# mratsim/constantine

Measured on NVIDIA H100. Metric: bls12_381_g1_msm_throughput, higher is better.
Workload: dtype u32

## Files before the change

### constantine_b200/csrc/msm_affine.cuh

```cuda
#pragma once
#include "ec.cuh"
#include "field_inv.cuh"

namespace b200 {

constexpr int AFF_MAX_LEVELS = 8;
constexpr uint32_t AFF_NONE = 0xFFFFFFFFu;

static __global__ void k_bucket_bounds(const uint32_t* __restrict__ keys, size_t n, uint32_t no_key, uint32_t* head, uint32_t* tail) {
  size_t q = (size_t)blockIdx.x * blockDim.x + threadIdx.x;
  if (q >= n) return;
  const uint32_t key = keys[q];
  if (key >= no_key) return;
  if (q == 0 || keys[q - 1] != key) head[key] = (uint32_t)q;
  if (q + 1 == n || keys[q + 1] != key) tail[key] = (uint32_t)(q + 1);
}

constexpr int SCAN_THREADS = 256, SCAN_PER_THREAD = 4, SCAN_ITEMS = SCAN_THREADS * SCAN_PER_THREAD;

B200_DEV uint32_t block_exclusive_scan(uint32_t v, uint32_t& total, uint32_t* smem ) {
  const unsigned lane = threadIdx.x & 31u, warp = threadIdx.x >> 5;
  uint32_t inc = v;
#pragma unroll
  for (int d = 1; d < 32; d <<= 1) {
// ... 3 lines not shown
  __syncthreads();
  if (lane == 31u) smem[warp] = inc;
  __syncthreads();
  uint32_t base = 0, tot = 0;
#pragma unroll
  for (int w = 0; w < SCAN_THREADS / 32; w++) {
    const uint32_t s = smem[w];
    if ((unsigned)w < warp) base += s;
    tot += s;
  }
  total = tot;
  return base + inc - v;
}

B200_DEV uint32_t level_count(uint32_t n, int r) { return (n + (1u << r) - 1u) >> r; }

static __global__ void __launch_bounds__(SCAN_THREADS) k_level_blocksums(const uint32_t* __restrict__ head, const uint32_t* __restrict__ tail,
                                                                          uint32_t nb, int L, uint32_t nblk, uint32_t* blocksum ) {
  __shared__ uint32_t sm[SCAN_THREADS / 32 + 1];
  const uint32_t b0 = blockIdx.x * SCAN_ITEMS + threadIdx.x * SCAN_PER_THREAD;
  uint32_t cnt[SCAN_PER_THREAD];
#pragma unroll
  for (int k = 0; k < SCAN_PER_THREAD; k++) cnt[k] = (b0 + k < nb) ? tail[b0 + k] - head[b0 + k] : 0u;
  for (int r = 0; r <= L; r++) {
    uint32_t s = 0;
#pragma unroll
    for (int k = 0; k < SCAN_PER_THREAD; k++) s += level_count(cnt[k], r);
    uint32_t tot;
    block_exclusive_scan(s, tot, sm);
    if (threadIdx.x == 0) blocksum[(size_t)r * nblk + blockIdx.x] = tot;
  }
}

static __global__ void __launch_bounds__(SCAN_THREADS) k_level_scan(uint32_t* blocksum, uint32_t nblk, int L, uint32_t nb, uint32_t* off) {
  __shared__ uint32_t sm[SCAN_THREADS / 32 + 1];
  for (int r = 0; r <= L; r++) {
    uint32_t carry = 0;
    for (uint32_t base = 0; base < nblk; base += SCAN_THREADS) {
      const uint32_t i = base + threadIdx.x;
      const uint32_t v = (i < nblk) ? blocksum[(size_t)r * nblk + i] : 0u;
      uint32_t tot;
      const uint32_t ex = block_exclusive_scan(v, tot, sm);
      if (i < nblk) blocksum[(size_t)r * nblk + i] = carry + ex;
      carry += tot;
    }
    if (threadIdx.x == 0) off[(size_t)r * (nb + 1) + nb] = carry;
  }
}

static __global__ void __launch_bounds__(SCAN_THREADS) k_level_offsets(const uint32_t* __restrict__ head, const uint32_t* __restrict__ tail,
                                                                        uint32_t nb, int L, uint32_t nblk, const uint32_t* __restrict__ blocksum,
                                                                        uint32_t* off) {
  __shared__ uint32_t sm[SCAN_THREADS / 32 + 1];
  const uint32_t b0 = blockIdx.x * SCAN_ITEMS + threadIdx.x * SCAN_PER_THREAD;
  uint32_t cnt[SCAN_PER_THREAD];
#pragma unroll
  for (int k = 0; k < SCAN_PER_THREAD; k++) cnt[k] = (b0 + k < nb) ? tail[b0 + k] - head[b0 + k] : 0u;
  for (int r = 0; r <= L; r++) {
    uint32_t c[SCAN_PER_THREAD], s = 0;
#pragma unroll
    for (int k = 0; k < SCAN_PER_THREAD; k++) { c[k] = level_count(cnt[k], r); s += c[k]; }
    uint32_t tot;
    uint32_t ex = block_exclusive_scan(s, tot, sm) + blocksum[(size_t)r * nblk + blockIdx.x];
#pragma unroll
    for (int k = 0; k < SCAN_PER_THREAD; k++) {
      if (b0 + k < nb) off[(size_t)r * (nb + 1) + b0 + k] = ex;
      ex += c[k];
    }
  }
}

struct AffinePlan {
  uint2* plan0;
  uint32_t* plan[AFF_MAX_LEVELS];
  uint32_t* surv_keys;
  uint32_t* surv_vals;
};

static __global__ void k_affine_plan(const uint32_t* __restrict__ keys, const uint32_t* __restrict__ vals, size_t n, uint32_t no_key,
                                     const uint32_t* __restrict__ head, const uint32_t* __restrict__ tail,
                                     const uint32_t* __restrict__ off, uint32_t nb, int L, AffinePlan P) {
  size_t q = (size_t)blockIdx.x * blockDim.x + threadIdx.x;
  if (q >= n) return;
  const uint32_t b = keys[q];
  if (b >= no_key) return;
  const uint32_t h = head[b], i = (uint32_t)q - h, cnt = tail[b] - h;
  const size_t stride = (size_t)nb + 1;
  for (int r = 0; r < L; r++) {
    if (i & ((2u << r) - 1u)) break;
    const uint32_t p = off[(size_t)(r + 1) * stride + b] + (i >> (r + 1));
    const uint32_t s = i >> r;
    const bool has2 = s + 1u < level_count(cnt, r);
    if (r == 0) P.plan0[p] = make_uint2(vals[q], has2 ? vals[q + 1] : AFF_NONE);
    else P.plan[r][p] = (off[(size_t)r * stride + b] + s) | (has2 ? 0x80000000u : 0u);
  }
  if ((i & ((1u << L) - 1u)) == 0u) {
    const uint32_t ps = off[(size_t)L * stride + b] + (i >> L);
    P.surv_keys[ps] = b;
    P.surv_vals[ps] = ps;
  }
}

template <class T>
B200_DEV Aff<T> load_affine_rw(const uint32_t* base, size_t idx) {
  const uint32_t* p = base + idx * (2 * T::WORDS);
  Aff<T> a;
  load_words_rw(a.x, p);
  load_words_rw(a.y, p + T::WORDS);
  return a;
// ... 18 lines not shown
template <class T>
B200_DEV T scratch_load(const uint4* scratch, size_t threads, size_t tid, uint32_t j) {
  constexpr int V = T::WORDS / 4;
  T v;
#pragma unroll
  for (int k = 0; k < V; k++) {
    const uint4 w = scratch[((size_t)j * V + k) * threads + tid];
    v.set_word(4 * k + 0, w.x); v.set_word(4 * k + 1, w.y); v.set_word(4 * k + 2, w.z); v.set_word(4 * k + 3, w.w);
  }
  return v;
}

constexpr int PART_TILE = 1024, PART_THREADS = 256, PART_MAX = 8;

B200_DEV uint32_t pair_chunk(const uint2 task, uint32_t n_points, uint32_t P) {
  uint32_t idx = task.x & 0x7FFFFFFFu;
  if (task.y != AFF_NONE) { const uint32_t j = task.y & 0x7FFFFFFFu; if (j > idx) idx = j; }
  uint32_t q = (uint32_t)(((unsigned long long)idx * P) / n_points);
  return q < P ? q : P - 1u;
}

static __global__ void __launch_bounds__(PART_THREADS) k_part_count(const uint2* __restrict__ plan0, const uint32_t* __restrict__ total_ptr,
                                                                    uint32_t n_points, uint32_t P, uint32_t nblk, uint32_t* counts) {
  __shared__ uint32_t sm[PART_MAX];
  if (threadIdx.x < PART_MAX) sm[threadIdx.x] = 0;
  __syncthreads();
  const uint32_t total = *total_ptr;
  const uint32_t base = blockIdx.x * PART_TILE;
  uint32_t local[PART_MAX];
#pragma unroll
  for (int q = 0; q < PART_MAX; q++) local[q] = 0;
  for (uint32_t i = threadIdx.x; i < PART_TILE; i += PART_THREADS) {
// ... 57 lines not shown
      for (unsigned w = 0; w < warp; w++) before += warp_cnt[w][q];
      perm[run_base[q] + before + my_rank] = p;
    }
    __syncthreads();
    if (threadIdx.x < P) {
      uint32_t tot = 0;
      for (unsigned w = 0; w < PART_THREADS / 32; w++) tot += warp_cnt[w][threadIdx.x];
      run_base[threadIdx.x] += tot;
    }
    __syncthreads();
  }
}

enum PairKind { PAIR_COPY1 = 0, PAIR_COPY2 = 1, PAIR_INF = 2, PAIR_ADD = 3, PAIR_DBL = 4 };

struct PairTask {
  uint32_t a, b;
};
template <bool FIRST>
B200_DEV PairTask load_task(const void* plan, size_t p) {
  PairTask t;
  if constexpr (FIRST) {
    const uint2 v = reinterpret_cast<const uint2*>(plan)[p];
    t.a = v.x; t.b = v.y;
  } else {
    const uint32_t v = reinterpret_cast<const uint32_t*>(plan)[p];
    t.a = v & 0x7FFFFFFFu;
    t.b = (v >> 31) ? t.a + 1u : AFF_NONE;
  }
  return t;
}
template <class T, bool FIRST>
B200_DEV T load_x(const uint32_t* src, uint32_t ref) {
  T x;
  if constexpr (FIRST) load_words(x, src + (size_t)(ref & 0x7FFFFFFFu) * (2 * T::WORDS));
  else load_words_rw(x, src + (size_t)ref * (2 * T::WORDS));
  return x;
}
template <class T, bool FIRST>
B200_DEV void decode_y(T& y, uint32_t ref, bool& zero) {
  zero = y.is_zero();
  if constexpr (FIRST) y.cneg((ref >> 31) != 0);
}
template <class T, bool FIRST>
B200_DEV T load_y(const uint32_t* src, uint32_t ref, bool& zero) {
  T y;
  if constexpr (FIRST) load_words(y, src + (size_t)(ref & 0x7FFFFFFFu) * (2 * T::WORDS) + T::WORDS);
  else load_words_rw(y, src + (size_t)ref * (2 * T::WORDS) + T::WORDS);
  decode_y<T, FIRST>(y, ref, zero);
  return y;
}

template <class T>
B200_DEV int classify_pair(bool single, const T& x1, const T& y1, bool inf1, const T& x2, const T& y2, bool inf2, T& den) {
  if (single) return PAIR_COPY1;
  if (inf1) return PAIR_COPY2;
  if (inf2) return PAIR_COPY1;
  den = x2 - x1;
  if (!den.is_zero()) return PAIR_ADD;
  if (!(y1 == y2) || y1.is_zero()) return PAIR_INF;
  den = y1.dbl();
  return PAIR_DBL;
}

template <class T, bool FIRST>
B200_DEV void pair_factor(const uint32_t* src, uint32_t a, uint32_t b, const T& x1, const T& x2, T& run) {
  const bool single = b == AFF_NONE;
  T den = x2 - x1;
  bool contributes = !single;
  if (!single && (den.is_zero() || x1.is_zero() || x2.is_zero())) {
    bool z1, z2;
    const T y1 = load_y<T, FIRST>(src, a, z1), y2 = load_y<T, FIRST>(src, b, z2);
    const int kind = classify_pair(false, x1, y1, z1 && x1.is_zero(), x2, y2, z2 && x2.is_zero(), den);
    contributes = kind >= PAIR_ADD;
  }
  if (contributes) run = run.mul_u(den);
}

template <class T, class Prefix>
B200_DEV Aff<T> pair_result(const Aff<T>& P1, bool z1, const Aff<T>& P2, bool z2, bool single, uint32_t j, T& inv, Prefix prefix) {
  T den;
  const int kind = classify_pair(single, P1.x, P1.y, z1 && P1.x.is_zero(), P2.x, P2.y, z2 && P2.x.is_zero(), den);
  Aff<T> R;
  if (kind < PAIR_ADD) {
    if (kind == PAIR_COPY1) R = P1;
    else if (kind == PAIR_COPY2) R = P2;
    else { R.x = T::zero(); R.y = T::zero(); }
  } else {
    T inv_den = inv;
    if (j > 0) inv_den = inv.mul_u(prefix());
    inv = inv.mul_u(den);
    T num;
    if (kind == PAIR_ADD) num = P2.y - P1.y;
    else { const T xx = P1.x.sqr(); num = xx.dbl() + xx; }
    const T lam = num.mul_u(inv_den);
    R.x = lam.sqr_u() - P1.x - P2.x;
    R.y = lam.mul_u(P1.x - R.x) - P1.y;
// ... 7 lines not shown
#ifndef B200_AFF_MIN_BLOCKS
#define B200_AFF_MIN_BLOCKS 4
#endif

B200_DEV void prefetch_l2(const void* p) { asm volatile("prefetch.global.L2 [%0];" ::"l"(p)); }
B200_DEV void prefetch_span(const void* p, int bytes) {
  prefetch_l2(p);
  prefetch_l2((const char*)p + bytes - 1);
}
template <class T, bool FIRST>
B200_DEV void prefetch_point(const uint32_t* src, uint32_t ref) {
  const uint32_t idx = FIRST ? (ref & 0x7FFFFFFFu) : ref;
  prefetch_span(src + (size_t)idx * (2 * T::WORDS), 2 * T::WORDS * 4);
}

__host__ __device__ __forceinline__ size_t pair_rows(size_t slots, size_t threads) { return (slots + threads - 1) / threads; }

struct PairSlots {
  const uint32_t* perm;
  uint32_t total, M;
  B200_DEV PairSlots(const uint32_t* total_ptr, const uint32_t* perm_, const uint32_t* range, size_t threads) {
    const uint32_t range_begin = range ? range[0] : 0u;
    total = range ? range[1] - range[0] : *total_ptr;
    perm = perm_;
    if (perm) perm += range_begin;
    M = (uint32_t)pair_rows(total, threads);
  }
  B200_DEV size_t first(size_t tid) const { return (tid & ~(size_t)31) * M + (tid & 31u); }
  B200_DEV uint32_t count(size_t tid) const {
    const size_t f = first(tid);
    if (f >= total) return 0u;
    const uint32_t c = (uint32_t)(((size_t)total - f + 31) / 32);
    return c < M ? c : M;
  }
  B200_DEV size_t slot(size_t tid, uint32_t j) const {
    const size_t t = first(tid) + 32u * (size_t)j;
    return perm ? (size_t)perm[t] : t;
  }
};

template <class T, bool FIRST>
__global__ void __launch_bounds__(B200_AFF_THREADS, (T::WORDS <= 12) ? B200_AFF_MIN_BLOCKS : 1)
k_affine_pairs(const void* __restrict__ plan, const uint32_t* __restrict__ total_ptr, const uint32_t* src, uint32_t* dst, uint4* scratch,
               const uint32_t* __restrict__ perm = nullptr, const uint32_t* __restrict__ range = nullptr) {
  const size_t threads = (size_t)gridDim.x * blockDim.x;
  const size_t tid = (size_t)blockIdx.x * blockDim.x + threadIdx.x;
  const PairSlots S(total_ptr, perm, range, threads);
  const unsigned lane = threadIdx.x & 31u;
  if (S.count(tid - lane) == 0) return;
  const uint32_t cnt = S.count(tid);
  T run = T::one();
  {
    PairTask t_next = cnt ? load_task<FIRST>(plan, S.slot(tid, 0)) : PairTask{0u, AFF_NONE};
    T x1n = T::zero(), x2n = T::zero();
    if (cnt) {
      x1n = load_x<T, FIRST>(src, t_next.a);
      if (t_next.b != AFF_NONE) x2n = load_x<T, FIRST>(src, t_next.b);
    }
#pragma unroll 1
    for (uint32_t j = 0; j < cnt; j++) {
      const PairTask t = t_next;
      const T x1 = x1n, x2 = x2n;
      if (j + 1 < cnt) {
        t_next = load_task<FIRST>(plan, S.slot(tid, j + 1));
        x1n = load_x<T, FIRST>(src, t_next.a);
        if (t_next.b != AFF_NONE) x2n = load_x<T, FIRST>(src, t_next.b);
      }
      pair_factor<T, FIRST>(src, t.a, t.b, x1, x2, run);
      scratch_store(scratch, threads, tid, j, run);
    }
  }
  T inv = fe_inverse(run);
  size_t p_prev = cnt ? S.slot(tid, cnt - 1) : 0;
  PairTask t_prev = cnt ? load_task<FIRST>(plan, p_prev) : PairTask{0u, AFF_NONE};
#pragma unroll 1
  for (uint32_t jj = cnt; jj > 0; jj--) {
    const uint32_t j = jj - 1;
    const size_t p = p_prev;
    const PairTask t = t_prev;
    if (j > 0) {
      p_prev = S.slot(tid, j - 1);
      t_prev = load_task<FIRST>(plan, p_prev);
      prefetch_point<T, FIRST>(src, t_prev.a);
      if (t_prev.b != AFF_NONE) prefetch_point<T, FIRST>(src, t_prev.b);
      if (j > 1) {
        constexpr int V = T::WORDS / 4;
#pragma unroll
        for (int k = 0; k < V; k++) prefetch_l2(scratch + ((size_t)(j - 2) * V + k) * threads + tid);
      }
    }
    const bool single = t.b == AFF_NONE;
    Aff<T> P1, P2;
    bool z1 = false, z2 = false;
    P1.x = load_x<T, FIRST>(src, t.a);
    P1.y = load_y<T, FIRST>(src, t.a, z1);
    if (!single) {
      P2.x = load_x<T, FIRST>(src, t.b);
      P2.y = load_y<T, FIRST>(src, t.b, z2);
    } else {
      P2.x = T::zero(); P2.y = T::zero();
    }
    store_affine(dst, p, pair_result(P1, z1, P2, z2, single, j, inv, [&] { return scratch_load<T>(scratch, threads, tid, j - 1); }));
  }
}

#ifndef B200_AFF_WS_CONSUMERS
#define B200_AFF_WS_CONSUMERS 8
#endif
#ifndef B200_AFF_WS_STAGES
#define B200_AFF_WS_STAGES 2
#endif
constexpr int AFF_WS_CONSUMERS = B200_AFF_WS_CONSUMERS;
constexpr int AFF_WS_THREADS = 32 * (AFF_WS_CONSUMERS + 1);

template <class T>
struct AffRing {
  static constexpr bool USED = T::WORDS <= 12;
  static constexpr int V = T::WORDS / 4;
// ... 24 lines not shown
  for (int k = 0; k < T::WORDS / 4; k++) cp_async16(ring + (row + k) * 32 + lane, g + 4 * k);
}
template <class T>
B200_DEV T ring_load(const uint4* ring, int row, unsigned lane) {
  T v;
#pragma unroll
  for (int k = 0; k < T::WORDS / 4; k++) {
    const uint4 w = ring[(row + k) * 32 + lane];
    v.set_word(4 * k + 0, w.x); v.set_word(4 * k + 1, w.y); v.set_word(4 * k + 2, w.z); v.set_word(4 * k + 3, w.w);
  }
  return v;
}

template <class T, bool FIRST>
__global__ void __launch_bounds__(AFF_WS_THREADS, 1)
k_affine_pairs_ws(const void* __restrict__ plan, const uint32_t* __restrict__ total_ptr, const uint32_t* src, uint32_t* dst, uint4* scratch,
                  const uint32_t* __restrict__ perm = nullptr, const uint32_t* __restrict__ range = nullptr) {
  using RG = AffRing<T>;
  constexpr int V = RG::V, NC = AFF_WS_CONSUMERS, S1 = RG::S1, S2 = RG::S2;
  extern __shared__ __align__(16) unsigned char aff_ring_raw[];
  __shared__ uint64_t full1[NC][S1], empty1[NC][S1], full2[NC][S2], empty2[NC][S2], drained[NC];
  __shared__ uint32_t s_task[NC][S1][3][32];
  const unsigned lane = threadIdx.x & 31u, warp = threadIdx.x >> 5;
  if (threadIdx.x == 0) {
    for (int w = 0; w < NC; w++) {
      for (int s = 0; s < S1; s++) { mbar_init(&full1[w][s], 64); mbar_init(&empty1[w][s], 32); }
      for (int s = 0; s < S2; s++) { mbar_init(&full2[w][s], 64); mbar_init(&empty2[w][s], 32); }
      mbar_init(&drained[w], 32);
    }
  }
  __syncthreads();
  const size_t threads = (size_t)gridDim.x * NC * 32;
  const PairSlots S(total_ptr, perm, range, threads);
  uint4* const ring_base = reinterpret_cast<uint4*>(aff_ring_raw);

  if (warp == NC) {
    uint32_t n[NC], cnt[NC];
#pragma unroll
    for (int w = 0; w < NC; w++) {
      const size_t tid = ((size_t)blockIdx.x * NC + w) * 32 + lane;
      n[w] = S.count(tid - lane);
      cnt[w] = S.count(tid);
    }
    auto tid_of = [&](int w) { return ((size_t)blockIdx.x * NC + w) * 32 + lane; };
    auto src_of = [&](uint32_t ref) { return src + (size_t)(FIRST ? (ref & 0x7FFFFFFFu) : ref) * (2 * T::WORDS); };
    uint32_t ta[NC], tb[NC], tp[NC];
    auto fetch_task = [&](int w, uint32_t j) {
      const size_t p = S.slot(tid_of(w), j);
      const PairTask t = load_task<FIRST>(plan, p);
      ta[w] = t.a; tb[w] = t.b; tp[w] = (uint32_t)p;
    };
#pragma unroll
    for (int w = 0; w < NC; w++) if (cnt[w]) fetch_task(w, 0);
#pragma unroll 1
    for (uint32_t j = 0; j < n[0]; j++) {
      uint32_t ca[NC], cb[NC];
#pragma unroll
      for (int w = 0; w < NC; w++) { ca[w] = ta[w]; cb[w] = tb[w]; }
#pragma unroll
      for (int w = 0; w < NC; w++) if (j + 1 < cnt[w]) fetch_task(w, j + 1);
#pragma unroll
      for (int w = 0; w < NC; w++) {
        if (j >= n[w]) continue;
        const int s = (int)(j % S1);
        mbar_wait(&empty1[w][s], ((j / S1) & 1u) ^ 1u);
        uint4* ring = ring_base + (size_t)w * RG::ROWS * 32;
        if (j < cnt[w]) {
          s_task[w][s][0][lane] = ca[w];
          s_task[w][s][1][lane] = cb[w];
          ring_fetch<T>(ring, s * 2 * V, lane, src_of(ca[w]));
          if (cb[w] != AFF_NONE) ring_fetch<T>(ring, s * 2 * V + V, lane, src_of(cb[w]));
        }
        cp_async_arrive(&full1[w][s]);
        mbar_arrive(&full1[w][s]);
      }
    }
#pragma unroll
    for (int w = 0; w < NC; w++) if (n[w] && n[w] - 1 < cnt[w]) fetch_task(w, n[w] - 1);
#pragma unroll 1
    for (uint32_t jj = 0; jj < n[0]; jj++) {
      uint32_t ca[NC], cb[NC], cp[NC];
#pragma unroll
      for (int w = 0; w < NC; w++) { ca[w] = ta[w]; cb[w] = tb[w]; cp[w] = tp[w]; }
#pragma unroll
      for (int w = 0; w < NC; w++) if (jj + 1 < n[w] && n[w] - 2 - jj < cnt[w]) fetch_task(w, n[w] - 2 - jj);
#pragma unroll
      for (int w = 0; w < NC; w++) {
        if (jj >= n[w]) continue;
        if (jj == 0) mbar_wait(&drained[w], 0);
        const uint32_t j = n[w] - 1 - jj;
        const int s = (int)(jj % S2);
        mbar_wait(&empty2[w][s], ((jj / S2) & 1u) ^ 1u);
        uint4* ring = ring_base + (size_t)w * RG::ROWS * 32;
        if (j < cnt[w]) {
          s_task[w][s][0][lane] = ca[w];
          s_task[w][s][1][lane] = cb[w];
          s_task[w][s][2][lane] = cp[w];
          const int row = s * 5 * V;
          ring_fetch<T>(ring, row, lane, src_of(ca[w]));
          ring_fetch<T>(ring, row + V, lane, src_of(ca[w]) + T::WORDS);
          if (cb[w] != AFF_NONE) {
            ring_fetch<T>(ring, row + 2 * V, lane, src_of(cb[w]));
            ring_fetch<T>(ring, row + 3 * V, lane, src_of(cb[w]) + T::WORDS);
          }
          if (j > 0) {
#pragma unroll
            for (int k = 0; k < V; k++)
              cp_async16(ring + (row + 4 * V + k) * 32 + lane, scratch + ((size_t)(j - 1) * V + k) * threads + tid_of(w));
          }
        }
        cp_async_arrive(&full2[w][s]);
        mbar_arrive(&full2[w][s]);
      }
    }
    asm volatile("cp.async.wait_all;" ::: "memory");
    return;
  }

  const size_t tid = ((size_t)blockIdx.x * NC + warp) * 32 + lane;
  const uint32_t n = S.count(tid - lane), cnt = S.count(tid);
  if (n == 0) return;
  const uint4* ring = ring_base + (size_t)warp * RG::ROWS * 32;
  T run = T::one();
#pragma unroll 1
  for (uint32_t j = 0; j < n; j++) {
    const int s = (int)(j % S1);
    mbar_wait(&full1[warp][s], (j / S1) & 1u);
    const uint32_t a = s_task[warp][s][0][lane], b = s_task[warp][s][1][lane];
    const T x1 = ring_load<T>(ring, s * 2 * V, lane), x2 = ring_load<T>(ring, s * 2 * V + V, lane);
    mbar_arrive(&empty1[warp][s]);
    if (j >= cnt) continue;
    pair_factor<T, FIRST>(src, a, b, x1, x2, run);
    scratch_store(scratch, threads, tid, j, run);
  }
  mbar_arrive(&drained[warp]);
  T inv = fe_inverse(run);
#pragma unroll 1
  for (uint32_t jj = 0; jj < n; jj++) {
    const uint32_t j = n - 1 - jj;
    const int s = (int)(jj % S2);
    mbar_wait(&full2[warp][s], (jj / S2) & 1u);
    const int row = s * 5 * V;
    const uint32_t a = s_task[warp][s][0][lane], b = s_task[warp][s][1][lane], p = s_task[warp][s][2][lane];
    const bool single = b == AFF_NONE;
    Aff<T> P1, P2;
    P1.x = ring_load<T>(ring, row, lane);
    P1.y = ring_load<T>(ring, row + V, lane);
    P2.x = single ? T::zero() : ring_load<T>(ring, row + 2 * V, lane);
    P2.y = single ? T::zero() : ring_load<T>(ring, row + 3 * V, lane);
    const T pre = ring_load<T>(ring, row + 4 * V, lane);
    mbar_arrive(&empty2[warp][s]);
    if (j >= cnt) continue;
    bool z1, z2 = false;
    decode_y<T, FIRST>(P1.y, a, z1);
    if (!single) decode_y<T, FIRST>(P2.y, b, z2);
    store_affine(dst, p, pair_result(P1, z1, P2, z2, single, j, inv, [&] { return pre; }));
  }
}

template <class T>
struct PairKernel {
  static constexpr bool WS = AffRing<T>::USED;
  static constexpr int THREADS = WS ? AFF_WS_THREADS : B200_AFF_THREADS;
  static constexpr int SLOT_THREADS = WS ? 32 * AFF_WS_CONSUMERS : B200_AFF_THREADS;
  static constexpr int SMEM = WS ? (int)AffRing<T>::BYTES : 0;
  template <bool FIRST>
  static auto entry() {
    if constexpr (WS) return k_affine_pairs_ws<T, FIRST>;
    else return k_affine_pairs<T, FIRST>;
  }
};

template <class T>
cudaError_t affine_pairs_blocks_per_sm(int* bps) {
  using K = PairKernel<T>;
  int b[2] = {0, 0};
  cudaError_t e;
  for (int f = 0; f < 2; f++) {
    const auto k = f == 0 ? K::template entry<true>() : K::template entry<false>();
    if (K::SMEM && (e = cudaFuncSetAttribute(k, cudaFuncAttributeMaxDynamicSharedMemorySize, K::SMEM)) != cudaSuccess) return e;
    if ((e = cudaOccupancyMaxActiveBlocksPerMultiprocessor(&b[f], k, K::THREADS, K::SMEM)) != cudaSuccess) return e;
  }
  *bps = b[1] < b[0] ? b[1] : b[0];
  return cudaSuccess;
}

template <class T, bool FIRST>
void launch_affine_pairs(unsigned grid, cudaStream_t s, const void* plan, const uint32_t* total_ptr, const uint32_t* src, uint32_t* dst, uint4* scratch,
                         const uint32_t* perm = nullptr, const uint32_t* range = nullptr) {
  using K = PairKernel<T>;
  K::template entry<FIRST>()<<<grid, K::THREADS, K::SMEM, s>>>(plan, total_ptr, src, dst, scratch, perm, range);
}

}
```

### constantine_b200/csrc/msm_engine.cuh

```cuda
#pragma once
#include <cstdio>
#include <cstdlib>
#include <cstring>
#include <atomic>
#include <condition_variable>
#include <functional>
#include <memory>
#include <mutex>
#include <thread>
#include <vector>
#include <cuda_runtime.h>
#include <cub/device/device_radix_sort.cuh>
#include <cub/device/device_scan.cuh>
#include "msm_kernels.cuh"
#include "msm_affine.cuh"
#include "host_field.hpp"

namespace b200 {

#define B200_CUDA_CHECK(expr)                                                                              \
  do {                                                                                                     \
    cudaError_t e__ = (expr);                                                                              \
    if (e__ != cudaSuccess) {                                                                              \
      fprintf(stderr, "[ctt_b200_msm] FATAL CUDA error %s (%s) at %s:%d -- no CPU fallback exists\n",      \
// ... 120 lines not shown
  int sm_count = 0;
  cudaStream_t stream = nullptr, copy_stream = nullptr;
  cudaStream_t user_stream = nullptr;
  cudaStream_t order_after = nullptr;
  cudaEvent_t ev_order = nullptr;
  cudaEvent_t ev_done = nullptr;
  bool unsynced = false, pending = false;
  cudaStream_t compute() const { return user_stream ? user_stream : stream; }
  cudaEvent_t msm_ev[MSM_MARKS];
  static constexpr int CALLER_MARKS = 6;
  cudaEvent_t caller_ev[CALLER_MARKS];
  cudaEvent_t ev_points_ready;
  static constexpr int MAX_INPUT_CHUNKS = 8;
  cudaEvent_t ev_chunk[MAX_INPUT_CHUNKS];
  DeviceBuffer d_scalars, d_points, keys_a, keys_b, vals_a, vals_b, cub_tmp, buckets, part_pts[2], part_keys[2], red_a, red_b, red_planes, bounds;
  DeviceBuffer aff_head, aff_tail, aff_off, aff_blocksum, aff_plan[AFF_MAX_LEVELS], aff_work[2], aff_scratch, keys_s, vals_s, part_counts, part_starts, part_perm;
  DeviceBuffer kzg_poly, kzg_args;
  DeviceBuffer das_coefs, das_cells, das_u, das_proofs;
  DeviceBuffer das_rec, das_z;
  DeviceBuffer ver_in, ver_pts, ver_aux;
  DeviceBuffer fft_data, fft_scratch, fft_tab;
  void* h_result = nullptr;
  size_t h_result_cap = 0;
  static constexpr size_t STAGE_BYTES = 16u << 20;
  void* h_stage[2] = {nullptr, nullptr};
  cudaEvent_t ev_stage[2] = {nullptr, nullptr};
  void ensure_stage() {
    if (h_stage[0]) return;
    for (int i = 0; i < 2; i++) {
      B200_CUDA_CHECK(cudaMallocHost(&h_stage[i], STAGE_BYTES));
      B200_CUDA_CHECK(cudaEventCreateWithFlags(&ev_stage[i], cudaEventDisableTiming));
// ... 295 lines not shown
  else if (ready) B200_CUDA_CHECK(cudaStreamWaitEvent(s, ready, 0));
}

template <class C>
void affine_levels(Engine& E, const MsmSizes& z, int AL, size_t entries, size_t acc_entries, size_t nper, const void* pts, int PC,
                   const PointChunks* pc, cudaEvent_t points_ready, bool timed, const uint32_t*& keys, const uint32_t*& vals,
                   const void*& acc_points, int& launches) {
  using T = typename C::T;
  constexpr size_t AFF_BYTES = 2 * T::WORDS * 4;
  cudaStream_t s = E.compute();
  auto level_cap = [&](int r) { return (entries >> r) + z.nbuckets + 1; };
  const uint32_t nb = (uint32_t)z.nbuckets;
  const uint32_t nblk = (nb + SCAN_ITEMS - 1) / SCAN_ITEMS;
  const size_t off_stride = (size_t)nb + 1;
  E.aff_head.ensure((size_t)nb * 4); E.aff_tail.ensure((size_t)nb * 4);
  E.aff_off.ensure((size_t)(AL + 1) * off_stride * 4);
  E.aff_blocksum.ensure((size_t)(AL + 1) * nblk * 4);
  E.aff_plan[0].ensure(level_cap(1) * 8);
  for (int r = 1; r < AL; r++) E.aff_plan[r].ensure(level_cap(r + 1) * 4);
  E.aff_work[1].ensure(level_cap(1) * AFF_BYTES);
  if (AL >= 2) E.aff_work[0].ensure(level_cap(2) * AFF_BYTES);
  E.keys_s.ensure(acc_entries * 4);
  E.vals_s.ensure(acc_entries * 4);
  static thread_local int bps_cache[MAX_DEVICES] = {};
  int bps = bps_cache[E.device];
  if (bps == 0) {
    B200_CUDA_CHECK(affine_pairs_blocks_per_sm<T>(&bps));
    if (bps < 1) bps = 1;
    bps_cache[E.device] = bps;
  }
  const unsigned aff_grid = (unsigned)(E.sm_count * bps);
  const size_t aff_threads = (size_t)aff_grid * PairKernel<T>::SLOT_THREADS;
  E.aff_scratch.ensure(pair_rows(level_cap(1), aff_threads) * aff_threads * (size_t)T::WORDS * 4);
  uint32_t* head = (uint32_t*)E.aff_head.ptr;
  uint32_t* tail = (uint32_t*)E.aff_tail.ptr;
  uint32_t* off = (uint32_t*)E.aff_off.ptr;
  B200_CUDA_CHECK(cudaMemsetAsync(head, 0, (size_t)nb * 4, s));
  B200_CUDA_CHECK(cudaMemsetAsync(tail, 0, (size_t)nb * 4, s));
  B200_CUDA_CHECK(cudaMemsetAsync(E.keys_s.ptr, 0xFF, acc_entries * 4, s));
  const unsigned eb = (unsigned)((entries + 255) / 256);
  k_bucket_bounds<<<eb, 256, 0, s>>>(keys, entries, z.no_key, head, tail);
  k_level_blocksums<<<nblk, SCAN_THREADS, 0, s>>>(head, tail, nb, AL, nblk, (uint32_t*)E.aff_blocksum.ptr);
  k_level_scan<<<1, SCAN_THREADS, 0, s>>>((uint32_t*)E.aff_blocksum.ptr, nblk, AL, nb, off);
  k_level_offsets<<<nblk, SCAN_THREADS, 0, s>>>(head, tail, nb, AL, nblk, (const uint32_t*)E.aff_blocksum.ptr, off);
  AffinePlan aplan;
  aplan.plan0 = (uint2*)E.aff_plan[0].ptr;
  for (int r = 0; r < AFF_MAX_LEVELS; r++) aplan.plan[r] = (r >= 1 && r < AL) ? (uint32_t*)E.aff_plan[r].ptr : nullptr;
  aplan.surv_keys = (uint32_t*)E.keys_s.ptr;
  aplan.surv_vals = (uint32_t*)E.vals_s.ptr;
  k_affine_plan<<<eb, 256, 0, s>>>(keys, vals, entries, z.no_key, head, tail, off, nb, AL, aplan);
  const bool split0 = PC > 1;
  if (!split0) wait_points(s, PC, pc, points_ready);
  for (int r = 0; r < AL; r++) {
    const uint32_t* total_ptr = off + (size_t)(r + 1) * off_stride + nb;
    uint32_t* dst = (uint32_t*)E.aff_work[(r + 1) & 1].ptr;
    if (r == 0 && split0) {
      const uint32_t Pq = (uint32_t)PC;
      const uint32_t nblk_p = (uint32_t)((level_cap(1) + PART_TILE - 1) / PART_TILE);
      E.part_counts.ensure((size_t)Pq * nblk_p * 4);
      E.part_starts.ensure((size_t)(Pq + 1) * 4);
      E.part_perm.ensure(level_cap(1) * 4);
      k_part_count<<<nblk_p, PART_THREADS, 0, s>>>((const uint2*)E.aff_plan[0].ptr, total_ptr, (uint32_t)nper, Pq, nblk_p, (uint32_t*)E.part_counts.ptr);
      k_part_scan<<<1, SCAN_THREADS, 0, s>>>((uint32_t*)E.part_counts.ptr, Pq, nblk_p, (uint32_t*)E.part_starts.ptr);
      k_part_scatter<<<nblk_p, PART_THREADS, 0, s>>>((const uint2*)E.aff_plan[0].ptr, total_ptr, (uint32_t)nper, Pq, nblk_p,
                                                      (const uint32_t*)E.part_counts.ptr, (uint32_t*)E.part_perm.ptr);
      for (int q = 0; q < PC; q++) {
        wait_piece(s, *pc, q);
        launch_affine_pairs<T, true>(aff_grid, s, E.aff_plan[0].ptr, total_ptr, (const uint32_t*)pts, dst, (uint4*)E.aff_scratch.ptr,
                                     (const uint32_t*)E.part_perm.ptr, (const uint32_t*)E.part_starts.ptr + q);
      }
      launches += 3 + PC - 1;
    } else if (r == 0)
      launch_affine_pairs<T, true>(aff_grid, s, E.aff_plan[0].ptr, total_ptr, (const uint32_t*)pts, dst, (uint4*)E.aff_scratch.ptr);
    else
      launch_affine_pairs<T, false>(aff_grid, s, E.aff_plan[r].ptr, total_ptr, (const uint32_t*)E.aff_work[r & 1].ptr, dst, (uint4*)E.aff_scratch.ptr);
  }
  keys = (const uint32_t*)E.keys_s.ptr;
  vals = (const uint32_t*)E.vals_s.ptr;
  acc_points = E.aff_work[AL & 1].ptr;
  k_window_bounds<<<(unsigned)((z.nw + 1 + 63) / 64), 64, 0, s>>>(keys, acc_entries, z.B, z.nw, (unsigned long long*)E.bounds.ptr);
  launches += 6 + AL;
  B200_CUDA_CHECK(cudaGetLastError());
  if (timed) B200_CUDA_CHECK(cudaEventRecord(E.msm_ev[MSM_AFFINE_DONE], s));
}

template <class C>
void msm_chunk(Engine& E, const MsmJob& job, const MsmSizes& z, const InputChunk& ch, bool chunked, bool into, bool timed, int& launches) {
  using T = typename C::T;
  constexpr int KFIX = 32;
  constexpr size_t XYZZ_BYTES = 4 * T::WORDS * 4;
// ... 714 lines not shown
```

Before: 115.1.

## Separate odd-bucket singletons from affine pair tasks into a copy list

The affine bucket-reduction plan now splits each level into true pairs and leftover single points. Singles go into a separate copy list with its own scanned offsets and count, while the pair list holds only real additions with an explicit output index. The batched-inversion kernels no longer spend inversion-chain slots, loads and divergent branches on single entries, and they copy singles in a simple loop at the end. In exchange the scan does twice as many rows, there are extra output-index and copy buffers, and there is an extra indirection load per pair.

```diff
diff --git a/constantine_b200/csrc/msm_affine.cuh b/constantine_b200/csrc/msm_affine.cuh
--- a/constantine_b200/csrc/msm_affine.cuh
+++ b/constantine_b200/csrc/msm_affine.cuh
@@ -5,7 +5,6 @@
 namespace b200 {
 
 constexpr int AFF_MAX_LEVELS = 8;
-constexpr uint32_t AFF_NONE = 0xFFFFFFFFu;
 
 static __global__ void k_bucket_bounds(const uint32_t* __restrict__ keys, size_t n, uint32_t no_key, uint32_t* head, uint32_t* tail) {
   size_t q = (size_t)blockIdx.x * blockDim.x + threadIdx.x;
@@ -41,6 +40,7 @@
 }
 
 B200_DEV uint32_t level_count(uint32_t n, int r) { return (n + (1u << r) - 1u) >> r; }
+B200_DEV uint32_t offset_row_count(uint32_t n, int row, int L) { return row <= L ? level_count(n, row) : level_count(n, row - L - 1) & 1u; }
 
 static __global__ void __launch_bounds__(SCAN_THREADS) k_level_blocksums(const uint32_t* __restrict__ head, const uint32_t* __restrict__ tail,
                                                                           uint32_t nb, int L, uint32_t nblk, uint32_t* blocksum ) {
@@ -49,29 +49,38 @@
   uint32_t cnt[SCAN_PER_THREAD];
 #pragma unroll
   for (int k = 0; k < SCAN_PER_THREAD; k++) cnt[k] = (b0 + k < nb) ? tail[b0 + k] - head[b0 + k] : 0u;
-  for (int r = 0; r <= L; r++) {
+  for (int row = 0; row <= 2 * L; row++) {
     uint32_t s = 0;
 #pragma unroll
-    for (int k = 0; k < SCAN_PER_THREAD; k++) s += level_count(cnt[k], r);
+    for (int k = 0; k < SCAN_PER_THREAD; k++) s += offset_row_count(cnt[k], row, L);
     uint32_t tot;
     block_exclusive_scan(s, tot, sm);
-    if (threadIdx.x == 0) blocksum[(size_t)r * nblk + blockIdx.x] = tot;
-  }
-}
-
-static __global__ void __launch_bounds__(SCAN_THREADS) k_level_scan(uint32_t* blocksum, uint32_t nblk, int L, uint32_t nb, uint32_t* off) {
+    if (threadIdx.x == 0) blocksum[(size_t)row * nblk + blockIdx.x] = tot;
+  }
+}
+
+static __global__ void __launch_bounds__(SCAN_THREADS) k_level_scan(uint32_t* blocksum, uint32_t nblk, int L, uint32_t nb, uint32_t* off,
+                                                                    uint32_t* counts) {
   __shared__ uint32_t sm[SCAN_THREADS / 32 + 1];
-  for (int r = 0; r <= L; r++) {
+  const size_t stride = (size_t)nb + 1;
+  for (int row = 0; row <= 2 * L; row++) {
     uint32_t carry = 0;
     for (uint32_t base = 0; base < nblk; base += SCAN_THREADS) {
       const uint32_t i = base + threadIdx.x;
-      const uint32_t v = (i < nblk) ? blocksum[(size_t)r * nblk + i] : 0u;
+      const uint32_t v = (i < nblk) ? blocksum[(size_t)row * nblk + i] : 0u;
       uint32_t tot;
       const uint32_t ex = block_exclusive_scan(v, tot, sm);
-      if (i < nblk) blocksum[(size_t)r * nblk + i] = carry + ex;
+      if (i < nblk) blocksum[(size_t)row * nblk + i] = carry + ex;
       carry += tot;
     }
-    if (threadIdx.x == 0) off[(size_t)r * (nb + 1) + nb] = carry;
+    if (threadIdx.x == 0) off[(size_t)row * stride + nb] = carry;
+  }
+  if (threadIdx.x == 0) {
+    for (int r = 0; r < L; r++) {
+      const uint32_t copies = off[(size_t)(L + 1 + r) * stride + nb];
+      counts[2 * r] = off[(size_t)(r + 1) * stride + nb] - copies;
+      counts[2 * r + 1] = copies;
+    }
   }
 }
 
@@ -83,23 +92,25 @@
   uint32_t cnt[SCAN_PER_THREAD];
 #pragma unroll
   for (int k = 0; k < SCAN_PER_THREAD; k++) cnt[k] = (b0 + k < nb) ? tail[b0 + k] - head[b0 + k] : 0u;
-  for (int r = 0; r <= L; r++) {
+  for (int row = 0; row <= 2 * L; row++) {
     uint32_t c[SCAN_PER_THREAD], s = 0;
 #pragma unroll
-    for (int k = 0; k < SCAN_PER_THREAD; k++) { c[k] = level_count(cnt[k], r); s += c[k]; }
+    for (int k = 0; k < SCAN_PER_THREAD; k++) { c[k] = offset_row_count(cnt[k], row, L); s += c[k]; }
     uint32_t tot;
-    uint32_t ex = block_exclusive_scan(s, tot, sm) + blocksum[(size_t)r * nblk + blockIdx.x];
+    uint32_t ex = block_exclusive_scan(s, tot, sm) + blocksum[(size_t)row * nblk + blockIdx.x];
 #pragma unroll
     for (int k = 0; k < SCAN_PER_THREAD; k++) {
-      if (b0 + k < nb) off[(size_t)r * (nb + 1) + b0 + k] = ex;
+      if (b0 + k < nb) off[(size_t)row * (nb + 1) + b0 + k] = ex;
       ex += c[k];
     }
   }
 }
 
 struct AffinePlan {
-  uint2* plan0;
-  uint32_t* plan[AFF_MAX_LEVELS];
+  uint2* pairs0;
+  uint32_t* pairs[AFF_MAX_LEVELS];
+  uint32_t* pair_out[AFF_MAX_LEVELS];
+  uint2* copies[AFF_MAX_LEVELS];
   uint32_t* surv_keys;
   uint32_t* surv_vals;
 };
@@ -117,9 +128,16 @@
     if (i & ((2u << r) - 1u)) break;
     const uint32_t p = off[(size_t)(r + 1) * stride + b] + (i >> (r + 1));
     const uint32_t s = i >> r;
-    const bool has2 = s + 1u < level_count(cnt, r);
-    if (r == 0) P.plan0[p] = make_uint2(vals[q], has2 ? vals[q + 1] : AFF_NONE);
-    else P.plan[r][p] = (off[(size_t)r * stride + b] + s) | (has2 ? 0x80000000u : 0u);
+    const uint32_t a = r == 0 ? vals[q] : off[(size_t)r * stride + b] + s;
+    const uint32_t singles_before = off[(size_t)(L + 1 + r) * stride + b];
+    if (s + 1u < level_count(cnt, r)) {
+      const uint32_t k = p - singles_before;
+      if (r == 0) P.pairs0[k] = make_uint2(a, vals[q + 1]);
+      else P.pairs[r][k] = a;
+      P.pair_out[r][k] = p;
+    } else {
+      P.copies[r][singles_before] = make_uint2(a, p);
+    }
   }
   if ((i & ((1u << L) - 1u)) == 0u) {
     const uint32_t ps = off[(size_t)L * stride + b] + (i >> L);
@@ -168,8 +186,7 @@
 constexpr int PART_TILE = 1024, PART_THREADS = 256, PART_MAX = 8;
 
 B200_DEV uint32_t pair_chunk(const uint2 task, uint32_t n_points, uint32_t P) {
-  uint32_t idx = task.x & 0x7FFFFFFFu;
-  if (task.y != AFF_NONE) { const uint32_t j = task.y & 0x7FFFFFFFu; if (j > idx) idx = j; }
+  const uint32_t idx = max(task.x & 0x7FFFFFFFu, task.y & 0x7FFFFFFFu);
   uint32_t q = (uint32_t)(((unsigned long long)idx * P) / n_points);
   return q < P ? q : P - 1u;
 }
@@ -257,19 +274,26 @@
 
 enum PairKind { PAIR_COPY1 = 0, PAIR_COPY2 = 1, PAIR_INF = 2, PAIR_ADD = 3, PAIR_DBL = 4 };
 
+struct PairLevel {
+  const void* pairs;
+  const uint32_t* out;
+  const uint32_t* npairs;
+  const uint2* copies;
+  const uint32_t* ncopies;
+};
+
 struct PairTask {
   uint32_t a, b;
 };
 template <bool FIRST>
-B200_DEV PairTask load_task(const void* plan, size_t p) {
+B200_DEV PairTask load_task(const void* pairs, size_t k) {
   PairTask t;
   if constexpr (FIRST) {
-    const uint2 v = reinterpret_cast<const uint2*>(plan)[p];
+    const uint2 v = reinterpret_cast<const uint2*>(pairs)[k];
     t.a = v.x; t.b = v.y;
   } else {
-    const uint32_t v = reinterpret_cast<const uint32_t*>(plan)[p];
-    t.a = v & 0x7FFFFFFFu;
-    t.b = (v >> 31) ? t.a + 1u : AFF_NONE;
+    t.a = reinterpret_cast<const uint32_t*>(pairs)[k];
+    t.b = t.a + 1u;
   }
   return t;
 }
@@ -295,8 +319,7 @@
 }
 
 template <class T>
-B200_DEV int classify_pair(bool single, const T& x1, const T& y1, bool inf1, const T& x2, const T& y2, bool inf2, T& den) {
-  if (single) return PAIR_COPY1;
+B200_DEV int classify_pair(const T& x1, const T& y1, bool inf1, const T& x2, const T& y2, bool inf2, T& den) {
   if (inf1) return PAIR_COPY2;
   if (inf2) return PAIR_COPY1;
   den = x2 - x1;
@@ -308,22 +331,21 @@
 
 template <class T, bool FIRST>
 B200_DEV void pair_factor(const uint32_t* src, uint32_t a, uint32_t b, const T& x1, const T& x2, T& run) {
-  const bool single = b == AFF_NONE;
   T den = x2 - x1;
-  bool contributes = !single;
-  if (!single && (den.is_zero() || x1.is_zero() || x2.is_zero())) {
+  bool contributes = true;
+  if (den.is_zero() || x1.is_zero() || x2.is_zero()) {
     bool z1, z2;
     const T y1 = load_y<T, FIRST>(src, a, z1), y2 = load_y<T, FIRST>(src, b, z2);
-    const int kind = classify_pair(false, x1, y1, z1 && x1.is_zero(), x2, y2, z2 && x2.is_zero(), den);
+    const int kind = classify_pair(x1, y1, z1 && x1.is_zero(), x2, y2, z2 && x2.is_zero(), den);
     contributes = kind >= PAIR_ADD;
   }
   if (contributes) run = run.mul_u(den);
 }
 
 template <class T, class Prefix>
-B200_DEV Aff<T> pair_result(const Aff<T>& P1, bool z1, const Aff<T>& P2, bool z2, bool single, uint32_t j, T& inv, Prefix prefix) {
+B200_DEV Aff<T> pair_result(const Aff<T>& P1, bool z1, const Aff<T>& P2, bool z2, uint32_t j, T& inv, Prefix prefix) {
   T den;
-  const int kind = classify_pair(single, P1.x, P1.y, z1 && P1.x.is_zero(), P2.x, P2.y, z2 && P2.x.is_zero(), den);
+  const int kind = classify_pair(P1.x, P1.y, z1 && P1.x.is_zero(), P2.x, P2.y, z2 && P2.x.is_zero(), den);
   Aff<T> R;
   if (kind < PAIR_ADD) {
     if (kind == PAIR_COPY1) R = P1;
@@ -361,7 +383,7 @@
   prefetch_span(src + (size_t)idx * (2 * T::WORDS), 2 * T::WORDS * 4);
 }
 
-__host__ __device__ __forceinline__ size_t pair_rows(size_t slots, size_t threads) { return (slots + threads - 1) / threads; }
+__host__ __device__ __forceinline__ size_t pair_rows(size_t pairs, size_t threads) { return (pairs + threads - 1) / threads; }
 
 struct PairSlots {
   const uint32_t* perm;
@@ -387,68 +409,84 @@
 };
 
 template <class T, bool FIRST>
+B200_DEV void copy_singles(const PairLevel& lv, const uint32_t* src, uint32_t* dst, size_t threads, size_t tid) {
+  if (!lv.copies) return;
+  const uint32_t n = *lv.ncopies;
+#pragma unroll 1
+  for (size_t k = tid; k < n; k += threads) {
+    const uint2 c = lv.copies[k];
+    Aff<T> P;
+    bool z;
+    P.x = load_x<T, FIRST>(src, c.x);
+    P.y = load_y<T, FIRST>(src, c.x, z);
+    store_affine(dst, c.y, P);
+  }
+}
+
+template <class T, bool FIRST>
 __global__ void __launch_bounds__(B200_AFF_THREADS, (T::WORDS <= 12) ? B200_AFF_MIN_BLOCKS : 1)
-k_affine_pairs(const void* __restrict__ plan, const uint32_t* __restrict__ total_ptr, const uint32_t* src, uint32_t* dst, uint4* scratch,
+k_affine_pairs(const PairLevel lv, const uint32_t* src, uint32_t* dst, uint4* scratch,
                const uint32_t* __restrict__ perm = nullptr, const uint32_t* __restrict__ range = nullptr) {
   const size_t threads = (size_t)gridDim.x * blockDim.x;
   const size_t tid = (size_t)blockIdx.x * blockDim.x + threadIdx.x;
-  const PairSlots S(total_ptr, perm, range, threads);
+  const PairSlots S(lv.npairs, perm, range, threads);
   const unsigned lane = threadIdx.x & 31u;
-  if (S.count(tid - lane) == 0) return;
+  if (S.count(tid - lane) == 0) {
+    copy_singles<T, FIRST>(lv, src, dst, threads, tid);
+    return;
+  }
   const uint32_t cnt = S.count(tid);
   T run = T::one();
   {
-    PairTask t_next = cnt ? load_task<FIRST>(plan, S.slot(tid, 0)) : PairTask{0u, AFF_NONE};
+    PairTask t_next = cnt ? load_task<FIRST>(lv.pairs, S.slot(tid, 0)) : PairTask{0u, 0u};
     T x1n = T::zero(), x2n = T::zero();
     if (cnt) {
       x1n = load_x<T, FIRST>(src, t_next.a);
-      if (t_next.b != AFF_NONE) x2n = load_x<T, FIRST>(src, t_next.b);
+      x2n = load_x<T, FIRST>(src, t_next.b);
     }
 #pragma unroll 1
     for (uint32_t j = 0; j < cnt; j++) {
       const PairTask t = t_next;
       const T x1 = x1n, x2 = x2n;
       if (j + 1 < cnt) {
-        t_next = load_task<FIRST>(plan, S.slot(tid, j + 1));
+        t_next = load_task<FIRST>(lv.pairs, S.slot(tid, j + 1));
         x1n = load_x<T, FIRST>(src, t_next.a);
-        if (t_next.b != AFF_NONE) x2n = load_x<T, FIRST>(src, t_next.b);
+        x2n = load_x<T, FIRST>(src, t_next.b);
       }
       pair_factor<T, FIRST>(src, t.a, t.b, x1, x2, run);
       scratch_store(scratch, threads, tid, j, run);
     }
   }
   T inv = fe_inverse(run);
-  size_t p_prev = cnt ? S.slot(tid, cnt - 1) : 0;
-  PairTask t_prev = cnt ? load_task<FIRST>(plan, p_prev) : PairTask{0u, AFF_NONE};
+  size_t k_prev = cnt ? S.slot(tid, cnt - 1) : 0;
+  PairTask t_prev = cnt ? load_task<FIRST>(lv.pairs, k_prev) : PairTask{0u, 0u};
+  uint32_t out_prev = cnt ? lv.out[k_prev] : 0u;
 #pragma unroll 1
   for (uint32_t jj = cnt; jj > 0; jj--) {
     const uint32_t j = jj - 1;
-    const size_t p = p_prev;
+    const uint32_t out = out_prev;
     const PairTask t = t_prev;
     if (j > 0) {
-      p_prev = S.slot(tid, j - 1);
-      t_prev = load_task<FIRST>(plan, p_prev);
+      k_prev = S.slot(tid, j - 1);
+      t_prev = load_task<FIRST>(lv.pairs, k_prev);
+      out_prev = lv.out[k_prev];
       prefetch_point<T, FIRST>(src, t_prev.a);
-      if (t_prev.b != AFF_NONE) prefetch_point<T, FIRST>(src, t_prev.b);
+      prefetch_point<T, FIRST>(src, t_prev.b);
       if (j > 1) {
         constexpr int V = T::WORDS / 4;
 #pragma unroll
         for (int k = 0; k < V; k++) prefetch_l2(scratch + ((size_t)(j - 2) * V + k) * threads + tid);
       }
     }
-    const bool single = t.b == AFF_NONE;
     Aff<T> P1, P2;
-    bool z1 = false, z2 = false;
+    bool z1, z2;
     P1.x = load_x<T, FIRST>(src, t.a);
     P1.y = load_y<T, FIRST>(src, t.a, z1);
-    if (!single) {
-      P2.x = load_x<T, FIRST>(src, t.b);
-      P2.y = load_y<T, FIRST>(src, t.b, z2);
-    } else {
-      P2.x = T::zero(); P2.y = T::zero();
-    }
-    store_affine(dst, p, pair_result(P1, z1, P2, z2, single, j, inv, [&] { return scratch_load<T>(scratch, threads, tid, j - 1); }));
-  }
+    P2.x = load_x<T, FIRST>(src, t.b);
+    P2.y = load_y<T, FIRST>(src, t.b, z2);
+    store_affine(dst, out, pair_result(P1, z1, P2, z2, j, inv, [&] { return scratch_load<T>(scratch, threads, tid, j - 1); }));
+  }
+  copy_singles<T, FIRST>(lv, src, dst, threads, tid);
 }
 
 #ifndef B200_AFF_WS_CONSUMERS
@@ -503,8 +541,7 @@
 
 template <class T, bool FIRST>
 __global__ void __launch_bounds__(AFF_WS_THREADS, 1)
-k_affine_pairs_ws(const void* __restrict__ plan, const uint32_t* __restrict__ total_ptr, const uint32_t* src, uint32_t* dst, uint4* scratch,
-                  const uint32_t* __restrict__ perm = nullptr, const uint32_t* __restrict__ range = nullptr) {
+k_affine_pairs_ws(const PairLevel lv, const uint32_t* src, uint32_t* dst, uint4* scratch, const uint32_t* __restrict__ perm = nullptr, const uint32_t* __restrict__ range = nullptr) {
   using RG = AffRing<T>;
   constexpr int V = RG::V, NC = AFF_WS_CONSUMERS, S1 = RG::S1, S2 = RG::S2;
   extern __shared__ __align__(16) unsigned char aff_ring_raw[];
@@ -520,7 +557,7 @@
   }
   __syncthreads();
   const size_t threads = (size_t)gridDim.x * NC * 32;
-  const PairSlots S(total_ptr, perm, range, threads);
+  const PairSlots S(lv.npairs, perm, range, threads);
   uint4* const ring_base = reinterpret_cast<uint4*>(aff_ring_raw);
 
   if (warp == NC) {
@@ -534,20 +571,21 @@
     auto tid_of = [&](int w) { return ((size_t)blockIdx.x * NC + w) * 32 + lane; };
     auto src_of = [&](uint32_t ref) { return src + (size_t)(FIRST ? (ref & 0x7FFFFFFFu) : ref) * (2 * T::WORDS); };
     uint32_t ta[NC], tb[NC], tp[NC];
-    auto fetch_task = [&](int w, uint32_t j) {
-      const size_t p = S.slot(tid_of(w), j);
-      const PairTask t = load_task<FIRST>(plan, p);
-      ta[w] = t.a; tb[w] = t.b; tp[w] = (uint32_t)p;
+    auto fetch_task = [&](int w, uint32_t j, bool with_out) {
+      const size_t k = S.slot(tid_of(w), j);
+      const PairTask t = load_task<FIRST>(lv.pairs, k);
+      ta[w] = t.a; tb[w] = t.b;
+      if (with_out) tp[w] = lv.out[k];
     };
 #pragma unroll
-    for (int w = 0; w < NC; w++) if (cnt[w]) fetch_task(w, 0);
+    for (int w = 0; w < NC; w++) if (cnt[w]) fetch_task(w, 0, false);
 #pragma unroll 1
     for (uint32_t j = 0; j < n[0]; j++) {
       uint32_t ca[NC], cb[NC];
 #pragma unroll
       for (int w = 0; w < NC; w++) { ca[w] = ta[w]; cb[w] = tb[w]; }
 #pragma unroll
-      for (int w = 0; w < NC; w++) if (j + 1 < cnt[w]) fetch_task(w, j + 1);
+      for (int w = 0; w < NC; w++) if (j + 1 < cnt[w]) fetch_task(w, j + 1, false);
 #pragma unroll
       for (int w = 0; w < NC; w++) {
         if (j >= n[w]) continue;
@@ -558,21 +596,21 @@
           s_task[w][s][0][lane] = ca[w];
           s_task[w][s][1][lane] = cb[w];
           ring_fetch<T>(ring, s * 2 * V, lane, src_of(ca[w]));
-          if (cb[w] != AFF_NONE) ring_fetch<T>(ring, s * 2 * V + V, lane, src_of(cb[w]));
+          ring_fetch<T>(ring, s * 2 * V + V, lane, src_of(cb[w]));
         }
         cp_async_arrive(&full1[w][s]);
         mbar_arrive(&full1[w][s]);
       }
     }
 #pragma unroll
-    for (int w = 0; w < NC; w++) if (n[w] && n[w] - 1 < cnt[w]) fetch_task(w, n[w] - 1);
+    for (int w = 0; w < NC; w++) if (n[w] && n[w] - 1 < cnt[w]) fetch_task(w, n[w] - 1, true);
 #pragma unroll 1
     for (uint32_t jj = 0; jj < n[0]; jj++) {
       uint32_t ca[NC], cb[NC], cp[NC];
 #pragma unroll
       for (int w = 0; w < NC; w++) { ca[w] = ta[w]; cb[w] = tb[w]; cp[w] = tp[w]; }
 #pragma unroll
-      for (int w = 0; w < NC; w++) if (jj + 1 < n[w] && n[w] - 2 - jj < cnt[w]) fetch_task(w, n[w] - 2 - jj);
+      for (int w = 0; w < NC; w++) if (jj + 1 < n[w] && n[w] - 2 - jj < cnt[w]) fetch_task(w, n[w] - 2 - jj, true);
 #pragma unroll
       for (int w = 0; w < NC; w++) {
         if (jj >= n[w]) continue;
@@ -588,10 +626,8 @@
           const int row = s * 5 * V;
           ring_fetch<T>(ring, row, lane, src_of(ca[w]));
           ring_fetch<T>(ring, row + V, lane, src_of(ca[w]) + T::WORDS);
-          if (cb[w] != AFF_NONE) {
-            ring_fetch<T>(ring, row + 2 * V, lane, src_of(cb[w]));
-            ring_fetch<T>(ring, row + 3 * V, lane, src_of(cb[w]) + T::WORDS);
-          }
+          ring_fetch<T>(ring, row + 2 * V, lane, src_of(cb[w]));
+          ring_fetch<T>(ring, row + 3 * V, lane, src_of(cb[w]) + T::WORDS);
           if (j > 0) {
 #pragma unroll
             for (int k = 0; k < V; k++)
@@ -608,7 +644,10 @@
 
   const size_t tid = ((size_t)blockIdx.x * NC + warp) * 32 + lane;
   const uint32_t n = S.count(tid - lane), cnt = S.count(tid);
-  if (n == 0) return;
+  if (n == 0) {
+    copy_singles<T, FIRST>(lv, src, dst, threads, tid);
+    return;
+  }
   const uint4* ring = ring_base + (size_t)warp * RG::ROWS * 32;
   T run = T::one();
 #pragma unroll 1
@@ -631,20 +670,20 @@
     mbar_wait(&full2[warp][s], (jj / S2) & 1u);
     const int row = s * 5 * V;
     const uint32_t a = s_task[warp][s][0][lane], b = s_task[warp][s][1][lane], p = s_task[warp][s][2][lane];
-    const bool single = b == AFF_NONE;
     Aff<T> P1, P2;
     P1.x = ring_load<T>(ring, row, lane);
     P1.y = ring_load<T>(ring, row + V, lane);
-    P2.x = single ? T::zero() : ring_load<T>(ring, row + 2 * V, lane);
-    P2.y = single ? T::zero() : ring_load<T>(ring, row + 3 * V, lane);
+    P2.x = ring_load<T>(ring, row + 2 * V, lane);
+    P2.y = ring_load<T>(ring, row + 3 * V, lane);
     const T pre = ring_load<T>(ring, row + 4 * V, lane);
     mbar_arrive(&empty2[warp][s]);
     if (j >= cnt) continue;
-    bool z1, z2 = false;
+    bool z1, z2;
     decode_y<T, FIRST>(P1.y, a, z1);
-    if (!single) decode_y<T, FIRST>(P2.y, b, z2);
-    store_affine(dst, p, pair_result(P1, z1, P2, z2, single, j, inv, [&] { return pre; }));
-  }
+    decode_y<T, FIRST>(P2.y, b, z2);
+    store_affine(dst, p, pair_result(P1, z1, P2, z2, j, inv, [&] { return pre; }));
+  }
+  copy_singles<T, FIRST>(lv, src, dst, threads, tid);
 }
 
 template <class T>
@@ -675,10 +714,10 @@
 }
 
 template <class T, bool FIRST>
-void launch_affine_pairs(unsigned grid, cudaStream_t s, const void* plan, const uint32_t* total_ptr, const uint32_t* src, uint32_t* dst, uint4* scratch,
+void launch_affine_pairs(unsigned grid, cudaStream_t s, const PairLevel& lv, const uint32_t* src, uint32_t* dst, uint4* scratch,
                          const uint32_t* perm = nullptr, const uint32_t* range = nullptr) {
   using K = PairKernel<T>;
-  K::template entry<FIRST>()<<<grid, K::THREADS, K::SMEM, s>>>(plan, total_ptr, src, dst, scratch, perm, range);
-}
-
-}
+  K::template entry<FIRST>()<<<grid, K::THREADS, K::SMEM, s>>>(lv, src, dst, scratch, perm, range);
+}
+
+}
diff --git a/constantine_b200/csrc/msm_engine.cuh b/constantine_b200/csrc/msm_engine.cuh
--- a/constantine_b200/csrc/msm_engine.cuh
+++ b/constantine_b200/csrc/msm_engine.cuh
@@ -158,7 +158,8 @@
   static constexpr int MAX_INPUT_CHUNKS = 8;
   cudaEvent_t ev_chunk[MAX_INPUT_CHUNKS];
   DeviceBuffer d_scalars, d_points, keys_a, keys_b, vals_a, vals_b, cub_tmp, buckets, part_pts[2], part_keys[2], red_a, red_b, red_planes, bounds;
-  DeviceBuffer aff_head, aff_tail, aff_off, aff_blocksum, aff_plan[AFF_MAX_LEVELS], aff_work[2], aff_scratch, keys_s, vals_s, part_counts, part_starts, part_perm;
+  DeviceBuffer aff_head, aff_tail, aff_off, aff_blocksum, aff_plan[AFF_MAX_LEVELS], aff_out[AFF_MAX_LEVELS], aff_copy[AFF_MAX_LEVELS], aff_work[2],
+      aff_scratch, keys_s, vals_s, part_counts, part_starts, part_perm;
   DeviceBuffer kzg_poly, kzg_args;
   DeviceBuffer das_coefs, das_cells, das_u, das_proofs;
   DeviceBuffer das_rec, das_z;
@@ -484,10 +485,13 @@
   const uint32_t nblk = (nb + SCAN_ITEMS - 1) / SCAN_ITEMS;
   const size_t off_stride = (size_t)nb + 1;
   E.aff_head.ensure((size_t)nb * 4); E.aff_tail.ensure((size_t)nb * 4);
-  E.aff_off.ensure((size_t)(AL + 1) * off_stride * 4);
-  E.aff_blocksum.ensure((size_t)(AL + 1) * nblk * 4);
-  E.aff_plan[0].ensure(level_cap(1) * 8);
-  for (int r = 1; r < AL; r++) E.aff_plan[r].ensure(level_cap(r + 1) * 4);
+  E.aff_off.ensure(((size_t)(2 * AL + 1) * off_stride + 2 * AL) * 4);
+  E.aff_blocksum.ensure((size_t)(2 * AL + 1) * nblk * 4);
+  for (int r = 0; r < AL; r++) {
+    E.aff_plan[r].ensure(level_cap(r + 1) * (r == 0 ? 8 : 4));
+    E.aff_out[r].ensure(level_cap(r + 1) * 4);
+    E.aff_copy[r].ensure((size_t)nb * 8);
+  }
   E.aff_work[1].ensure(level_cap(1) * AFF_BYTES);
   if (AL >= 2) E.aff_work[0].ensure(level_cap(2) * AFF_BYTES);
   E.keys_s.ensure(acc_entries * 4);
@@ -501,28 +505,33 @@
   }
   const unsigned aff_grid = (unsigned)(E.sm_count * bps);
   const size_t aff_threads = (size_t)aff_grid * PairKernel<T>::SLOT_THREADS;
-  E.aff_scratch.ensure(pair_rows(level_cap(1), aff_threads) * aff_threads * (size_t)T::WORDS * 4);
+  E.aff_scratch.ensure(pair_rows(entries / 2, aff_threads) * aff_threads * (size_t)T::WORDS * 4);
   uint32_t* head = (uint32_t*)E.aff_head.ptr;
   uint32_t* tail = (uint32_t*)E.aff_tail.ptr;
   uint32_t* off = (uint32_t*)E.aff_off.ptr;
+  uint32_t* counts = off + (size_t)(2 * AL + 1) * off_stride;
   B200_CUDA_CHECK(cudaMemsetAsync(head, 0, (size_t)nb * 4, s));
   B200_CUDA_CHECK(cudaMemsetAsync(tail, 0, (size_t)nb * 4, s));
   B200_CUDA_CHECK(cudaMemsetAsync(E.keys_s.ptr, 0xFF, acc_entries * 4, s));
   const unsigned eb = (unsigned)((entries + 255) / 256);
   k_bucket_bounds<<<eb, 256, 0, s>>>(keys, entries, z.no_key, head, tail);
   k_level_blocksums<<<nblk, SCAN_THREADS, 0, s>>>(head, tail, nb, AL, nblk, (uint32_t*)E.aff_blocksum.ptr);
-  k_level_scan<<<1, SCAN_THREADS, 0, s>>>((uint32_t*)E.aff_blocksum.ptr, nblk, AL, nb, off);
+  k_level_scan<<<1, SCAN_THREADS, 0, s>>>((uint32_t*)E.aff_blocksum.ptr, nblk, AL, nb, off, counts);
   k_level_offsets<<<nblk, SCAN_THREADS, 0, s>>>(head, tail, nb, AL, nblk, (const uint32_t*)E.aff_blocksum.ptr, off);
   AffinePlan aplan;
-  aplan.plan0 = (uint2*)E.aff_plan[0].ptr;
-  for (int r = 0; r < AFF_MAX_LEVELS; r++) aplan.plan[r] = (r >= 1 && r < AL) ? (uint32_t*)E.aff_plan[r].ptr : nullptr;
+  aplan.pairs0 = (uint2*)E.aff_plan[0].ptr;
+  for (int r = 0; r < AFF_MAX_LEVELS; r++) {
+    aplan.pairs[r] = (r >= 1 && r < AL) ? (uint32_t*)E.aff_plan[r].ptr : nullptr;
+    aplan.pair_out[r] = r < AL ? (uint32_t*)E.aff_out[r].ptr : nullptr;
+    aplan.copies[r] = r < AL ? (uint2*)E.aff_copy[r].ptr : nullptr;
+  }
   aplan.surv_keys = (uint32_t*)E.keys_s.ptr;
   aplan.surv_vals = (uint32_t*)E.vals_s.ptr;
   k_affine_plan<<<eb, 256, 0, s>>>(keys, vals, entries, z.no_key, head, tail, off, nb, AL, aplan);
   const bool split0 = PC > 1;
   if (!split0) wait_points(s, PC, pc, points_ready);
   for (int r = 0; r < AL; r++) {
-    const uint32_t* total_ptr = off + (size_t)(r + 1) * off_stride + nb;
+    const PairLevel lv{E.aff_plan[r].ptr, (const uint32_t*)E.aff_out[r].ptr, counts + 2 * r, (const uint2*)E.aff_copy[r].ptr, counts + 2 * r + 1};
     uint32_t* dst = (uint32_t*)E.aff_work[(r + 1) & 1].ptr;
     if (r == 0 && split0) {
       const uint32_t Pq = (uint32_t)PC;
@@ -530,20 +539,22 @@
       E.part_counts.ensure((size_t)Pq * nblk_p * 4);
       E.part_starts.ensure((size_t)(Pq + 1) * 4);
       E.part_perm.ensure(level_cap(1) * 4);
-      k_part_count<<<nblk_p, PART_THREADS, 0, s>>>((const uint2*)E.aff_plan[0].ptr, total_ptr, (uint32_t)nper, Pq, nblk_p, (uint32_t*)E.part_counts.ptr);
+      k_part_count<<<nblk_p, PART_THREADS, 0, s>>>((const uint2*)E.aff_plan[0].ptr, lv.npairs, (uint32_t)nper, Pq, nblk_p, (uint32_t*)E.part_counts.ptr);
       k_part_scan<<<1, SCAN_THREADS, 0, s>>>((uint32_t*)E.part_counts.ptr, Pq, nblk_p, (uint32_t*)E.part_starts.ptr);
-      k_part_scatter<<<nblk_p, PART_THREADS, 0, s>>>((const uint2*)E.aff_plan[0].ptr, total_ptr, (uint32_t)nper, Pq, nblk_p,
+      k_part_scatter<<<nblk_p, PART_THREADS, 0, s>>>((const uint2*)E.aff_plan[0].ptr, lv.npairs, (uint32_t)nper, Pq, nblk_p,
                                                       (const uint32_t*)E.part_counts.ptr, (uint32_t*)E.part_perm.ptr);
       for (int q = 0; q < PC; q++) {
         wait_piece(s, *pc, q);
-        launch_affine_pairs<T, true>(aff_grid, s, E.aff_plan[0].ptr, total_ptr, (const uint32_t*)pts, dst, (uint4*)E.aff_scratch.ptr,
+        PairLevel piece = lv;
+        if (q + 1 < PC) piece.copies = nullptr;
+        launch_affine_pairs<T, true>(aff_grid, s, piece, (const uint32_t*)pts, dst, (uint4*)E.aff_scratch.ptr,
                                      (const uint32_t*)E.part_perm.ptr, (const uint32_t*)E.part_starts.ptr + q);
       }
       launches += 3 + PC - 1;
     } else if (r == 0)
-      launch_affine_pairs<T, true>(aff_grid, s, E.aff_plan[0].ptr, total_ptr, (const uint32_t*)pts, dst, (uint4*)E.aff_scratch.ptr);
+      launch_affine_pairs<T, true>(aff_grid, s, lv, (const uint32_t*)pts, dst, (uint4*)E.aff_scratch.ptr);
     else
-      launch_affine_pairs<T, false>(aff_grid, s, E.aff_plan[r].ptr, total_ptr, (const uint32_t*)E.aff_work[r & 1].ptr, dst, (uint4*)E.aff_scratch.ptr);
+      launch_affine_pairs<T, false>(aff_grid, s, lv, (const uint32_t*)E.aff_work[r & 1].ptr, dst, (uint4*)E.aff_scratch.ptr);
   }
   keys = (const uint32_t*)E.keys_s.ptr;
   vals = (const uint32_t*)E.vals_s.ptr;
```

After: 120.5 (median of 6 runs). 1.05x the previous value.
